# xxxxxxyp/Light-3D-Unet-Front

Measured on AMD Instinct MI355X. Metric: train patches/sec (48³, bs=4/GPU) at 1/2/4/8 MI355X + fwd ms/patch, higher is better.
Workload: dtype fp32; 1 GPU; Lightweight3DUNet 16->32->64->128 train step (fwd+FocalTversky+bwd+AdamW), 48^3 patches; batch_per_gpu=4, global_batch=4, ftl_mode=exact, parallelism=single, graph=True

## Files before the change

### include/l3u.h

```cpp
#ifndef L3U_H
#define L3U_H

#include <hip/hip_runtime.h>

#ifdef __cplusplus
extern "C" {
#endif

typedef unsigned short l3u_bf16;

#define L3U_ABI_VERSION 5
int l3u_abi_version(void);

typedef struct l3u_norm_src {
  const float* stat_part;
  int nsb;
  int layer;
  const float* gamma;
  const float* beta;
  float drop_p;
  unsigned long long seed;
  const int* step;
  float* rec_out;
  const float* rank1;
// ... 76 lines not shown
                    float drop_p, unsigned long long seed, const int* step, int layer, float* rec,
                    int N, int C, hipStream_t stream);
int l3u_norm_act_nblocks(int S);
int l3u_norm_act_fwd(const float* y2, long long y2_nstride, const float* rec2,
                     const l3u_norm_src* src2, const float* r, long long r_nstride,
                     const float* rec_r, const l3u_norm_src* src_r, int shortcut, float* out,
                     long long out_nstride, int N, int C, int S, hipStream_t stream);
int l3u_norm_act_pool_fwd(const float* y2, long long y2_nstride, const float* rec2,
                          const l3u_norm_src* src2, const float* r, long long r_nstride,
                          const float* rec_r, const l3u_norm_src* src_r, int shortcut, float* out,
                          long long out_nstride, float* pooled, long long pooled_nstride,
                          unsigned char* idx, int N, int C, int D, int H, int W,
                          hipStream_t stream);
int l3u_norm_act_bwd_reduce(const float* dout, long long dout_nstride, const float* out,
                            long long out_nstride, const float* y2, long long y2_nstride,
                            const float* rec2, const float* r, long long r_nstride,
                            const float* rec_r, double* part, int N, int C, int S,
                            hipStream_t stream);
int l3u_norm_act_bwd_reduce_r1(const float* dz, long long dz_nstride, const float* dscale,
                               const float* out, long long out_nstride, const float* y2,
                               long long y2_nstride, const float* rec2, const float* r,
                               long long r_nstride, const float* rec_r, double* part, int N, int C,
                               int S, hipStream_t stream);
int l3u_norm_act_bwd_reduce_up(const float* dskip, long long dskip_nstride, const float* dpool,
                               long long dpool_nstride, const unsigned char* idx, const float* out,
                               long long out_nstride, const float* y2, long long y2_nstride,
                               const float* rec2, const float* r, long long r_nstride,
                               const float* rec_r, double* part, int N, int C, int D, int H, int W,
                               hipStream_t stream);
int l3u_norm_act_bwd_apply(const float* dout, long long dout_nstride, const float* out,
                           long long out_nstride, const float* y2, long long y2_nstride,
                           const float* rec2, const float* r, long long r_nstride,
                           const float* rec_r, const double* part, float* dy2,
                           long long dy2_nstride, float* dr, long long dr_nstride, int N, int C,
                           int S, hipStream_t stream);
int l3u_norm_act_bwd(const float* dout, long long dout_nstride, const float* out,
                     long long out_nstride, const float* y2, long long y2_nstride,
                     const float* rec2, const float* r, long long r_nstride, const float* rec_r,
                     double* part, float* dy2, long long dy2_nstride, float* dr,
                     long long dr_nstride, int N, int C, int S, hipStream_t stream);
int l3u_norm_act_bwd_up(const float* dskip, long long dskip_nstride, const float* dpool,
                        long long dpool_nstride, const unsigned char* idx, const float* out,
                        long long out_nstride, const float* y2, long long y2_nstride,
                        const float* rec2, const float* r, long long r_nstride,
                        const float* rec_r, double* part, float* dy2, long long dy2_nstride,
                        float* dr, long long dr_nstride, int N, int C, int D, int H, int W,
// ... 439 lines not shown
```

### light-3d-unet-front_amd/csrc/misc.hip

```cpp
#include "common.h"
#ifdef L3U_STAMP
#include <vector>
#endif
using namespace l3u;

typedef float f4 __attribute__((ext_vector_type(4)));

namespace {

template <typename T>
__global__ __launch_bounds__(256) void maxpool2_fwd_kernel(
    const T* __restrict__ x, long long xns, T* __restrict__ y, long long yns,
    unsigned char* __restrict__ idx, int C, int D, int H, int W) {
  L3U_STAMP_SCOPE(401);
  const int Do = D / 2, Ho = H / 2, Wo = W / 2;
  const long long So = (long long)Do * Ho * Wo, Si = (long long)D * H * W;
  const int nc = blockIdx.y, c = nc % C, n = nc / C;
  const T* xp = x + (long long)n * xns + (long long)c * Si;
  T* yp = y + (long long)n * yns + (long long)c * So;
  unsigned char* ip = idx + (long long)nc * So;
  for (long long o = blockIdx.x * 256ll + threadIdx.x; o < So; o += (long long)gridDim.x * 256) {
    const int ox = (int)(o % Wo), t = (int)(o / Wo), oy = t % Ho, oz = t / Ho;
    const T* b = xp + ((long long)(2 * oz) * H + 2 * oy) * W + 2 * ox;
    float best = ld1(b);
// ... 85 lines not shown
#pragma unroll
  for (int q = 0; q < 4; ++q) {
    if (i0 + q < S) {
      const float tv = VEC ? tv4[q] : t[(long long)n * S + i0 + q];
      spt = fmaf(pv[q], tv, spt);
      sp += pv[q];
      st += tv;
      if (L4) se += bce_term(pv[q], tv);
    }
  }
  spt = block_sum256(spt, red);
  sp = block_sum256(sp, red);
  st = block_sum256(st, red);
  if (L4) se = block_sum256(se, red);
  if (threadIdx.x == 0) {
    float* o = ftl_part + ((long long)n * gridDim.x + blockIdx.x) * (L4 ? 4 : 3);
    o[0] = spt;
    o[1] = sp;
    o[2] = st;
    if (L4) o[3] = se;
  }
}

struct FtlCoef { double loss, A, B; };

L3U_DEV FtlCoef ftl_coef(const double* sums, double alpha, double beta, double gamma, double smooth) {
  const double tp = sums[0], fp = sums[1] - sums[0], fn = sums[2] - sums[0];
  const double dn = tp + alpha * fn + beta * fp + smooth;
  const double ti = (tp + smooth) / dn;
  const double one_m = 1.0 - ti;
  FtlCoef r;
  r.loss = pow(one_m, gamma);
  const double pre = -gamma * pow(one_m, gamma - 1.0) / (dn * dn);
  r.A = pre * (dn - (tp + smooth) * (1.0 - alpha));
  r.B = pre * (-(tp + smooth) * beta);
  return r;
}

L3U_DEV void ftl_lane_sums(const float* __restrict__ part, int nb, double& a, double& b, double& c) {
  const int l = threadIdx.x & 63;
  a = b = c = 0.0;
  constexpr int B = 8;
  for (int i = l; i < nb; i += B * 64) {
    float va[B], vb[B], vc[B];
#pragma unroll
    for (int u = 0; u < B; ++u) {
      const int j = min(i + u * 64, nb - 1);
      va[u] = part[j * 3];
      vb[u] = part[j * 3 + 1];
      vc[u] = part[j * 3 + 2];
    }
#pragma unroll
    for (int u = 0; u < B; ++u) {
      const bool ok = i + u * 64 < nb;
      a += ok ? va[u] : 0.f;
      b += ok ? vb[u] : 0.f;
      c += ok ? vc[u] : 0.f;
    }
  }
  a = wave_sum_d(a);
  b = wave_sum_d(b);
  c = wave_sum_d(c);
}

L3U_DEV void loss4_lane_sums(const float* __restrict__ part, int nb, double* sm) {
  const int l = threadIdx.x & 63;
  double a = 0.0, b = 0.0, c = 0.0, d = 0.0;
  constexpr int B = 8;
  for (int i = l; i < nb; i += B * 64) {
    float va[B], vb[B], vc[B], vd[B];
#pragma unroll
    for (int u = 0; u < B; ++u) {
      const int j = min(i + u * 64, nb - 1);
      va[u] = part[j * 4];
      vb[u] = part[j * 4 + 1];
      vc[u] = part[j * 4 + 2];
      vd[u] = part[j * 4 + 3];
    }
#pragma unroll
    for (int u = 0; u < B; ++u) {
      const bool ok = i + u * 64 < nb;
      a += ok ? va[u] : 0.f;
      b += ok ? vb[u] : 0.f;
      c += ok ? vc[u] : 0.f;
      d += ok ? vd[u] : 0.f;
    }
// ... 59 lines not shown
    }
#pragma unroll
    for (int c = 0; c < 32; ++c) {
      hv[c] = f4{0.f, 0.f, 0.f, 0.f};
      if (c < C && i0 < S) hv[c] = ldv4(hp + (long long)c * S + i0);
    }
  }
  float cA = 0.f, cB = 0.f, cE = 0.f;
  if (L4 && dp == nullptr) {
    double sm[4];
    if (fpart != nullptr) {
      loss4_lane_sums(fpart, fnp, sm);
    } else {
      sm[0] = sums[0]; sm[1] = sums[1]; sm[2] = sums[2]; sm[3] = sums[3];
    }
    const Loss4Coef r = loss4_coef(sm, fam);
    const double s = gscale ? (double)gscale[0] : 1.0;
    cA = (float)(r.A * s);
    cB = (float)(r.B * s);
    cE = (float)(r.E * s);
    if (loss && blockIdx.x == 0 && blockIdx.y == 0 && threadIdx.x == 0) loss[0] = (float)r.loss;
  }
  if (!L4 && dp == nullptr) {
    double sm[3];
    if (fpart != nullptr) {
      ftl_lane_sums(fpart, fnp, sm[0], sm[1], sm[2]);
    } else {
      sm[0] = sums[0]; sm[1] = sums[1]; sm[2] = sums[2];
    }
    const FtlCoef r = ftl_coef(sm, alpha, beta, gamma, smooth);
    const double s = gscale ? (double)gscale[0] : 1.0;
    cA = (float)(r.A * s);
    cB = (float)(r.B * s);
    if (loss && blockIdx.x == 0 && blockIdx.y == 0 && threadIdx.x == 0) loss[0] = (float)r.loss;
  }
  f4 dz = {0.f, 0.f, 0.f, 0.f};
#pragma unroll
  for (int q = 0; q < 4; ++q) {
    if (i0 + q < S) {
      const float pv = VEC ? pv4[q] : p[o + i0 + q];
      const float gs = VEC ? gv4[q] : (dp ? dp[o + i0 + q] : t[o + i0 + q]);
      const float g = dp ? gs : (L4 ? loss4_grad(cA - cB, cB, cE, pv, gs) : fmaf(cA - cB, gs, cB));
      dz[q] = g * pv * (1.f - pv);
    }
  }
  float acc[33];
#pragma unroll
  for (int c = 0; c < 33; ++c) acc[c] = 0.f;
  acc[32] = (dz[0] + dz[1]) + (dz[2] + dz[3]);
  if (dz_only) {
    if (VEC) {
      if (i0 < S) stv4(dhp + i0, dz);
    } else {
#pragma unroll
      for (int q = 0; q < 4; ++q)
        if (i0 + q < S) st1(dhp + i0 + q, dz[q]);
    }
  }
#pragma unroll
  for (int c = 0; c < 32; ++c) {
    if (c < C) {
      if (VEC) {
        if (i0 < S) {
          const f4 hc = hv[VEC ? c : 0];
          acc[c] = fmaf(dz[0], hc[0], fmaf(dz[1], hc[1], fmaf(dz[2], hc[2], dz[3] * hc[3])));
          if (!dz_only) stv4(dhp + (long long)c * S + i0, w[c] * dz);
        }
      } else {
#pragma unroll
        for (int q = 0; q < 4; ++q)
          if (i0 + q < S) {
            acc[c] = fmaf(dz[q], ld1(hp + (long long)c * S + i0 + q), acc[c]);
            if (!dz_only) st1(dhp + (long long)c * S + i0 + q, w[c] * dz[q]);
          }
      }
    }
  }
  const int wv = threadIdx.x >> 6, l = threadIdx.x & 63;
#pragma unroll
  for (int c = 0; c < 33; ++c) {
    if (c < C || c == 32) {
      const double r = wave_sum_d((double)acc[c]);
      if (l == 0) redd[wv * (C + 1) + (c == 32 ? C : c)] = r;
    }
  }
  __syncthreads();
  if (threadIdx.x <= C) {
    const int tt = threadIdx.x;
// ... 856 lines not shown
```

### light-3d-unet-front_amd/csrc/norm.hip

```cpp
#include "common.h"
using namespace l3u;

typedef float f4 __attribute__((ext_vector_type(4)));

namespace {

__global__ __launch_bounds__(256) void in_finalize_kernel(l3u_norm_src src, int NC, int C) {
  L3U_STAMP_SCOPE(301);
  const int wid = blockIdx.x * 4 + (threadIdx.x >> 6), l = threadIdx.x & 63;
  if (wid >= NC) return;
  float r[kRec];
  finalize_record(src, wid / C, wid % C, C, r);
  if (l == 0) {
    float* o = src.rec_out + (long long)wid * kRec;
#pragma unroll
    for (int i = 0; i < kRec; ++i) o[i] = r[i];
  }
}

template <typename T, bool VEC, bool HAS_SRC, bool RK = false>
__global__ __launch_bounds__(256) void norm_act_fwd_kernel(
    const T* __restrict__ y2, long long y2ns, const float* __restrict__ rec2, l3u_norm_src src2,
    const T* __restrict__ r, long long rns, const float* __restrict__ recr, l3u_norm_src srcr,
    int shortcut, T* __restrict__ out, long long ons, int C, int S) {
// ... 116 lines not shown
      stv4(op + off, v[j]);
      v[j] = round_to(v[j], (const T*)nullptr);
    }
    float b0 = v[0][0], b1 = v[0][2];
    int i0 = 0, i1 = 0;
#pragma unroll
    for (int j = 0; j < 4; ++j)
#pragma unroll
      for (int dx = 0; dx < 2; ++dx) {
        if (j == 0 && dx == 0) continue;
        const float u0 = v[j][dx], u1 = v[j][2 + dx];
        if (u0 > b0 || u0 != u0) { b0 = u0; i0 = 2 * j + dx; }
        if (u1 > b1 || u1 != u1) { b1 = u1; i1 = 2 * j + dx; }
      }
    stv2(pp + 2 * o, f2_t{b0, b1});
    ip[o] = (unsigned short)(i0 | (i1 << 8));
  }
}

#ifndef L3U_NABR_U
#define L3U_NABR_U 2
#endif
constexpr int kNabrU = L3U_NABR_U;
template <typename T, bool VEC, bool RK = false, bool PL = false>
__global__ __launch_bounds__(256) void norm_act_bwd_reduce_kernel(
    const float* __restrict__ dout, long long dns, const T* __restrict__ out, long long ons,
    const T* __restrict__ y2, long long y2ns, const float* __restrict__ rec2,
    const T* __restrict__ r, long long rns, const float* __restrict__ recr,
    double* __restrict__ part, int N, int C, int S, const float* __restrict__ dscale = nullptr,
    const float* __restrict__ dpool = nullptr, long long dpns = 0,
    const unsigned char* __restrict__ pidx = nullptr, int H = 0, int W = 0) {
  L3U_STAMP_SCOPE(304);
  kargs_now(dout, dns, out, ons, y2, y2ns, rec2, r, rns, recr, part, N, C, S, dscale, dpool, dpns,
            pidx, H, W);
  __shared__ double red[4];
  const int nc = blockIdx.y, c = nc % C, n = nc / C, nb = gridDim.x;
  const float m2 = rec2[(long long)nc * kRec + 0], rs2 = rec2[(long long)nc * kRec + 1];
  float mr = 0.f, rsr = 1.f, rks = 1.f;
  if (recr) {
    mr = recr[(long long)nc * kRec + 0]; rsr = recr[(long long)nc * kRec + 1];
    rks = recr[(long long)nc * kRec + 7];
  }
  constexpr bool rk = RK;
  const long long co = (long long)c * S;
  const float* dp = dout + (long long)n * dns + (dscale ? 0 : co);
  const float dsc = dscale ? dscale[c] : 1.f;
  const T* op = out + (long long)n * ons + co;
  const T* yp = y2 + (long long)n * y2ns + co;
  const T* rp = r + (long long)n * (rk ? -rns : rns) + (rk ? 0ll : co);
  double s0 = 0.0, s1 = 0.0, s2 = 0.0;
  if (VEC) {
    constexpr int U = kNabrU;
    const int step = nb * 1024;
    const T* rq = recr ? rp : op;
    for (int i0 = (blockIdx.x * 256 + threadIdx.x) * 4; i0 < S; i0 += U * step) {
      f4 ov[U], dv[U], yv[U], rv[U];
      UnpoolTap pt[U];
      int zz[U], yy[U];
#pragma unroll
      for (int u = 0; u < U; ++u) {
        const int i = min(i0 + u * step, S - 4);
        ov[u] = ldv4(op + i);
        dv[u] = ldv4(dp + i);
        yv[u] = ldv4(yp + i);
        rv[u] = ldv4(rq + i);
      }
      if constexpr (PL) {
#pragma unroll
        for (int u = 0; u < U; ++u) {
          const int i = min(i0 + u * step, S - 4);
          const int HW = H * W, z = fdiv(i, HW, 1.f / HW), rm = i - z * HW, y = fdiv(rm, W, 1.f / W);
          zz[u] = z; yy[u] = y;
          pt[u] = unpool_tap(dpool + (long long)n * dpns + (long long)c * (S / 8),
                             pidx + (long long)nc * (S / 8), z, y, rm - y * W, H, W);
        }
      }
      __builtin_amdgcn_sched_barrier(0);
#pragma unroll
      for (int u = 0; u < U; ++u) {
        dv[u] = dsc * dv[u];
        if constexpr (PL) dv[u] = unpool_apply(dv[u], pt[u], zz[u], yy[u]);
        if (rk) rv[u] = mul_rn(rv[u], rks);
      }
#pragma unroll
      for (int u = 0; u < U; ++u) {
        const bool in = u == 0 || i0 + u * step < S;
#pragma unroll
        for (int q = 0; q < 4; ++q) {
          const float g = dv[u][q] * lrelu_d(ov[u][q]);
          const double t1 = (double)g * ((yv[u][q] - m2) * rs2);
          const double t2 = (double)g * ((rv[u][q] - mr) * rsr);
          s0 = in ? s0 + g : s0;
          s1 = in ? s1 + t1 : s1;
          if (recr) s2 = in ? s2 + t2 : s2;
        }
      }
    }
  } else {
    for (int i = blockIdx.x * 256 + threadIdx.x; i < S; i += nb * 256) {
      const float g = (dscale ? dsc * ld1(dp + i) : ld1(dp + i)) * lrelu_d(ld1(op + i));
      s0 += g;
      s1 += (double)g * ((ld1(yp + i) - m2) * rs2);
      if (recr) s2 += (double)g * (((rk ? mul_rn(rks, ld1(rp + i)) : ld1(rp + i)) - mr) * rsr);
    }
  }
  s0 = block_sum256d(s0, red);
  s1 = block_sum256d(s1, red);
  s2 = block_sum256d(s2, red);
  if (threadIdx.x == 0) {
// ... 331 lines not shown
                             const float* rec_r, double* part, int N, int C, int S,
                             hipStream_t stream, const float* dscale = nullptr,
                             const float* dpool = nullptr, long long dpns = 0,
                             const unsigned char* pidx = nullptr, int H = 0, int W = 0) {
  L3U_REQUIRE(N > 0 && C > 0 && S > 0);
  L3U_REQUIRE(r_nstride >= 0 || (sizeof(T) == 4 && rec_r != nullptr));
  const bool vec = S % 4 == 0 && dout_nstride % 4 == 0 && out_nstride % 4 == 0 &&
                   y2_nstride % 4 == 0 && r_nstride % 4 == 0;
  L3U_REQUIRE(dpool == nullptr || (vec && pidx && H % 2 == 0 && W % 4 == 0 && (S / (H * W)) % 2 == 0 &&
                                   dpns % 2 == 0 && ((uintptr_t)dpool & 7) == 0));
  dim3 grid(elem_blocks(S), N * C);
  L3U_REQUIRE(r_nstride >= 0 || vec);
#define NABR(RK_, PL_) hipLaunchKernelGGL((norm_act_bwd_reduce_kernel<T, true, RK_, PL_>), grid, dim3(256), 0, \
      stream, dout, dout_nstride, out, out_nstride, y2, y2_nstride, rec2, r, r_nstride, rec_r, part, N, C, S, \
      dscale, dpool, dpns, pidx, H, W)
  if (r_nstride < 0) {
    if constexpr (sizeof(T) == 4) { if (dpool) NABR(true, true); else NABR(true, false); }
  } else if (vec) { if (dpool) NABR(false, true); else NABR(false, false); }
#undef NABR
  else hipLaunchKernelGGL((norm_act_bwd_reduce_kernel<T, false>), grid, dim3(256), 0, stream, dout, dout_nstride, out, out_nstride, y2, y2_nstride, rec2, r, r_nstride, rec_r, part, N, C, S, dscale);
  L3U_CHECK_LAUNCH();
}

template <typename T>
int norm_act_bwd_apply_impl(const float* dout, long long dout_nstride, const T* out,
                            long long out_nstride, const T* y2, long long y2_nstride,
                            const float* rec2, const T* r, long long r_nstride,
                            const float* rec_r, const double* part, float* dy2,
                            long long dy2_nstride, float* dr, long long dr_nstride, int N, int C,
                            int S, hipStream_t stream) {
  L3U_REQUIRE(N > 0 && C > 0 && S > 0);
  L3U_REQUIRE(r_nstride >= 0);
  const bool vec = S % 4 == 0 && dout_nstride % 4 == 0 && out_nstride % 4 == 0 &&
                   y2_nstride % 4 == 0 && r_nstride % 4 == 0 && dy2_nstride % 4 == 0 &&
                   dr_nstride % 4 == 0;
  const int npart = elem_blocks(S);
  dim3 grid(npart, N * C);
  if (vec) hipLaunchKernelGGL((norm_act_bwd_apply_kernel<T, true>), grid, dim3(256), 0, stream, dout, dout_nstride, out, out_nstride, y2, y2_nstride, rec2, r, r_nstride, rec_r, part, npart, dy2, dy2_nstride, dr, dr_nstride, N, C, S);
  else hipLaunchKernelGGL((norm_act_bwd_apply_kernel<T, false>), grid, dim3(256), 0, stream, dout, dout_nstride, out, out_nstride, y2, y2_nstride, rec2, r, r_nstride, rec_r, part, npart, dy2, dy2_nstride, dr, dr_nstride, N, C, S);
  L3U_CHECK_LAUNCH();
}

template <typename T>
int norm_act_bwd_impl(const float* dout, long long dout_nstride, const T* out,
                      long long out_nstride, const T* y2, long long y2_nstride,
                      const float* rec2, const T* r, long long r_nstride, const float* rec_r,
// ... 41 lines not shown
    int C, int D, int H, int W, hipStream_t stream)
L3U_TWIN(l3u_norm_act_pool_fwd, P_NAP, norm_act_pool_fwd_impl(bp(y2), y2_nstride, rec2, src2, bp(r),
         r_nstride, rec_r, src_r, shortcut, bp(out), out_nstride, bp(pooled), pooled_nstride, idx, N,
         C, D, H, W, stream))
#define P_NBR(TT) (const float* dout, long long dout_nstride, const TT* out, long long out_nstride,   \
    const TT* y2, long long y2_nstride, const float* rec2, const TT* r, long long r_nstride,        \
    const float* rec_r, double* part, int N, int C, int S, hipStream_t stream)
L3U_TWIN(l3u_norm_act_bwd_reduce, P_NBR, norm_act_bwd_reduce_impl(dout, dout_nstride, bp(out),
         out_nstride, bp(y2), y2_nstride, rec2, bp(r), r_nstride, rec_r, part, N, C, S, stream))
#define P_NBR1(TT) (const float* dz, long long dz_nstride, const float* dscale, const TT* out,        \
    long long out_nstride, const TT* y2, long long y2_nstride, const float* rec2, const TT* r,       \
    long long r_nstride, const float* rec_r, double* part, int N, int C, int S, hipStream_t stream)
#define P_NBRU(TT) (const float* dskip, long long dskip_nstride, const float* dpool,                  \
    long long dpool_nstride, const unsigned char* idx, const TT* out, long long out_nstride,         \
    const TT* y2, long long y2_nstride, const float* rec2, const TT* r, long long r_nstride,        \
    const float* rec_r, double* part, int N, int C, int D, int H, int W, hipStream_t stream)
L3U_TWIN(l3u_norm_act_bwd_reduce_up, P_NBRU, dpool == nullptr ? (int)hipErrorInvalidValue :
         norm_act_bwd_reduce_impl(dskip, dskip_nstride, bp(out), out_nstride, bp(y2), y2_nstride, rec2,
         bp(r), r_nstride, rec_r, part, N, C, D * H * W, stream, nullptr, dpool, dpool_nstride, idx, H,
         W))
L3U_TWIN(l3u_norm_act_bwd_reduce_r1, P_NBR1, dscale == nullptr ? (int)hipErrorInvalidValue :
         norm_act_bwd_reduce_impl(dz, dz_nstride, bp(out), out_nstride, bp(y2), y2_nstride, rec2, bp(r),
         r_nstride, rec_r, part, N, C, S, stream, dscale))
#define P_NBA(TT) (const float* dout, long long dout_nstride, const TT* out, long long out_nstride,   \
    const TT* y2, long long y2_nstride, const float* rec2, const TT* r, long long r_nstride,        \
    const float* rec_r, const double* part, float* dy2, long long dy2_nstride, float* dr,          \
    long long dr_nstride, int N, int C, int S, hipStream_t stream)
L3U_TWIN(l3u_norm_act_bwd_apply, P_NBA, norm_act_bwd_apply_impl(dout, dout_nstride, bp(out),
         out_nstride, bp(y2), y2_nstride, rec2, bp(r), r_nstride, rec_r, part, dy2, dy2_nstride,
         dr, dr_nstride, N, C, S, stream))
#define P_NB1(TT) (const float* dout, long long dout_nstride, const TT* out, long long out_nstride,   \
    const TT* y2, long long y2_nstride, const float* rec2, const TT* r, long long r_nstride,        \
    const float* rec_r, double* part, float* dy2, long long dy2_nstride, float* dr,                 \
    long long dr_nstride,                                                                            \
    int N, int C, int S, hipStream_t stream)
L3U_TWIN(l3u_norm_act_bwd, P_NB1, norm_act_bwd_impl(dout, dout_nstride, bp(out), out_nstride,
         bp(y2), y2_nstride, rec2, bp(r), r_nstride, rec_r, part, dy2, dy2_nstride, dr,
         dr_nstride, N, C, S, stream))
#define P_NB1U(TT) (const float* dskip, long long dskip_nstride, const float* dpool,                 \
    long long dpool_nstride, const unsigned char* idx, const TT* out, long long out_nstride,         \
    const TT* y2, long long y2_nstride, const float* rec2, const TT* r, long long r_nstride,        \
    const float* rec_r, double* part, float* dy2, long long dy2_nstride, float* dr,                 \
    long long dr_nstride, int N, int C, int D, int H, int W, hipStream_t stream)
L3U_TWIN(l3u_norm_act_bwd_up, P_NB1U, dpool == nullptr ? (int)hipErrorInvalidValue :
         norm_act_bwd_impl(dskip, dskip_nstride, bp(out), out_nstride, bp(y2), y2_nstride, rec2,
         bp(r), r_nstride, rec_r, part, dy2, dy2_nstride, dr, dr_nstride, N, C, D * H * W, stream,
// ... 8 lines not shown
```

### light-3d-unet-front_amd/light_unet/_native.py

```python
import ctypes
import os
import warnings

import torch

_HERE = os.path.dirname(os.path.abspath(__file__))
LIB_PATH = os.environ.get(
    "L3U_LIB", os.path.join(os.path.dirname(_HERE), "lib", "libl3u_hip.so"))

ABI_VERSION = 5

P = ctypes.c_void_p
I = ctypes.c_int
L = ctypes.c_longlong
F = ctypes.c_float
D = ctypes.c_double
U64 = ctypes.c_ulonglong

_FAM = [D] * 9

_SIGS = {
    "l3u_abi_version": [],
    "l3u_dw3_nchunk": [I, I, I, I, I],
    "l3u_dw3_fwd": [P, L, P, P, P, P, L, I, I, I, I, I, P],
# ... 48 lines not shown
    "l3u_gconv3_fwd": [P, L, P, P, P, L, P, I, I, I, I, I, I, I, P],
    "l3u_gconv3_bwd_data": [P, L, P, P, P, L, P, L, I, P, I, I, I, I, I, I, I, P],
    "l3u_gconv3_bwd_weight": [P, L, P, L, P, P, I, I, I, I, I, I, I, P],
    "l3u_counter_add": [P, I, P],
    "l3u_cast_f32_bf16": [P, P, L, P],
    "l3u_box_copy": [P, L, I, I, I, P, L, I, I, I, I, I, I, I, I, P],
    "l3u_ccl_nchunks": [L],
    "l3u_aug_patches": [P, I, I, I, I, P, P, P, P, P, P],
    "l3u_aug_draw": [P, P, I, D, U64, P, I, I, I, I, P, P, P, P, P],
    "l3u_ccl_label": [P, F, P, P, P, I, I, I, P],
    "l3u_ccl_stats": [P, P, P, P, I, I, I, I, P],
    "l3u_ccl_pairs": [P, P, I, P, L, P],
    "l3u_ccl_label_b": [P, F, P, P, P, I, I, I, I, P],
    "l3u_ccl_stats_b": [P, P, P, P, I, I, I, I, I, I, P],
    "l3u_ccl_lv_max_levels": [L, L],
    "l3u_thr_levels": [P, P, P, P, I, P, P, P, L, P],
    "l3u_ccl_label_lv": [P, I, I, P, P, P, P, I, I, I, P],
    "l3u_ccl_stats_lv": [P, P, P, P, I, I, I, I, I, P],
    "l3u_ccl_pairs_lv": [P, P, I, P, P, I, L, P],
    "l3u_cast_bf16_f32": [P, P, L, P],
    "l3u_outconv_bwd_dz": [P, P, P, P, D, D, D, D, P, P, L, P, P, L, P, P, I, I, I, P],
    "l3u_outconv_bwd_ftl_dz": [P, P, P, I, D, D, D, D, P, P, L, P, P, L, P, P, I, I, I, P],
    "l3u_norm_act_bwd_reduce_r1": [P, L, P, P, L, P, L, P, P, L, P, P, I, I, I, P],
    "l3u_pw_bwd_tail_r1": [P, L, P, P, L, P, L, P, P, I, I, P, L, P, P, L, I, P, I, I, I, I, P],
    "l3u_norm_act_bwd_reduce_up": [P, L, P, L, P, P, L, P, L, P, P, L, P, P, I, I, I, I, I, P],
    "l3u_pw_bwd_tail_up": [P, L, P, L, P, P, L, P, L, P, P, I, I, P, L, P, P, L, I, P, I, I, I, I, I, I,
                           P],
    "l3u_dwpw_supported": [I, I, I, I, I, I],
    "l3u_dw3_bwd_rank1": [I, I, I, I, I],
    "l3u_dwpw_stat_nsb": [I, I, I, I, I],
    "l3u_dwpw_fwd": [P, L, P, P, P, P, P, L, P, P, P, L, P, P, L, I, I, I, I, I, I, P],
    "l3u_loss4_sums": [P, P, L, P, P, P],
    "l3u_loss4_reduce": [P, I, P, P],
    "l3u_loss4_value": [P] + _FAM + [P, P],
    "l3u_loss4_bwd": [P, P, L, P] + _FAM + [P, I, P, P],
    "l3u_outconv_fwd_loss4": [P, L, P, P, P, P, P, I, I, I, P],
    "l3u_outconv_bwd_loss4": [P, P, P] + _FAM + [P, P, L, P, P, L, P, P, I, I, I, P],
    "l3u_outconv_bwd_loss4_dz": [P, P, P] + _FAM + [P, P, L, P, P, L, P, P, I, I, I, P],
    "l3u_outconv_bwd_loss4p": [P, P, P, I] + _FAM + [P, P, L, P, P, L, P, P, I, I, I, P],
    "l3u_outconv_bwd_loss4p_dz": [P, P, P, I] + _FAM + [P, P, L, P, P, L, P, P, I, I, I, P],
    "l3u_pp_select_ws_bytes": [],
    "l3u_pp_select": [P, I, L, I, L, L, L, L, P, P, P],
    "l3u_pp_normalize": [P, I, P, D, D, D, P, P, P, I, I, I, P],
    "l3u_pp_pack": [P, I, I, D, P, I, I, I, P],
    "l3u_pp_unpack": [P, P, I, I, I, I, P],
    "l3u_pp_morph_max_iters": [I],
# ... 139 lines not shown
```

### light-3d-unet-front_amd/light_unet/engine.py

```python
import math
import os

import torch

from . import _native as nat

F32 = 4
_FRONT = os.environ.get("L3U_FRONT", "1") != "0"
_PAIR_PW = os.environ.get("L3U_PAIR_PW", "1") != "0"
_TAIL_FUSE = os.environ.get("L3U_TAIL_FUSE", "1") != "0"
_SEG_CAPS = tuple(int(v) for v in os.environ.get("L3U_SEG_CAPS", "128,64,32").split(","))
_SEG_SHORT = tuple(int(v) for v in os.environ.get("L3U_SEG_SHORT", "32:256").split(":"))
_DWPW = os.environ.get("L3U_DWPW", "1") != "0"
_PAIR_BWD = os.environ.get("L3U_PAIR_BWD", "1") != "0"
_PAIR_TAIL_MAX_S = int(os.environ.get("L3U_PAIR_TAIL_MAX_S", str(48 ** 3)))
_PAIR_TAIL_NARROW = os.environ.get("L3U_PAIR_TAIL_NARROW", "1") != "0"
_DWPW_MIN_S = int(os.environ.get("L3U_DWPW_MIN_S", "65536"))
_RANK1 = os.environ.get("L3U_RANK1", "1") != "0"
_POOLFOLD = os.environ.get("L3U_POOLFOLD", "1") != "0"
_FRONT_R1 = os.environ.get("L3U_FRONT_R1", "1") != "0"
_FUSE_ADAMW = os.environ.get("L3U_FUSE_ADAMW", "1") != "0"


_SEG_SORT = os.environ.get("L3U_SEG_SORT", "1") != "0"


def _seg_rounds(it):
    src, cnt, ist, tst, ln, _, _, f64 = it
    vec = not f64 and tst == 1 and ln % 4 == 0 and ist % 4 == 0 and src % 4 == 0
    tp = 256 // (ln // 4) if vec else 256 // ln
    return -(-(-(-cnt // tp)) // 8)


def _items_cover_once(items, numel):
    cnt = torch.zeros(numel, dtype=torch.int32)
    for it in items:
        if it[6]:
            return False
        cnt[it[5]:it[5] + it[4]] += 1
    return bool((cnt == 1).all())


class V:
    __slots__ = ("t", "off", "ns", "C", "scale", "pool")

    def __init__(self, t, off, ns, C, scale=None, pool=None):
        self.t, self.off, self.ns, self.C, self.scale = t, off, ns, C, scale
        self.pool = pool

    @property
    def p(self):
        return self.t.data_ptr() + self.t.element_size() * self.off

    @property
    def sns(self):
        return -self.ns if self.scale is not None else self.ns


def conv_kinds(cin, cout, use_depthwise_separable=True, use_grouped=True, groups=8):
    if use_depthwise_separable:
        return ("ds", 0), ("ds", 0)
    k1 = ("grouped", groups) if (use_grouped and groups > 1 and cin >= groups and cout >= groups) \
        else ("dense", 1)
    k2 = ("grouped", groups) if (use_grouped and groups > 1 and cout >= groups) else ("dense", 1)
    return k1, k2


def _conv_params(pre, kind, cin, cout):
    if kind[0] == "ds":
        return [(pre + "depthwise.weight", (cin, 1, 3, 3, 3)),
# ... 537 lines not shown
        else:
            nat.call("l3u_reduce_segments", self.bwd_arena.ptr(0), items.data_ptr(),
                     items.shape[0], gflat.data_ptr(), nat.stream())
        return dx

    def _backward_impl(self, flat, gflat, sv, dp, need_dx, ftl=None, family=None):
        N = sv["N"]
        dims, S = sv["dims"], sv["S"]
        c0, c1, c2, c3 = self.enc
        dev = sv["p"].device
        e = lambda *s: self._empty(*s, device=dev)
        st = nat.stream()
        A = self.bwd_arena
        h = sv["h"]
        up3 = sv["blk"]["up3.res_block."]
        r1 = _RANK1 and self.kinds["up3.res_block."][0][0] == "ds" and \
            self._tail_fusable(up3, up3["x"].C, c0, S[0])
        sfx = "_dz" if r1 else ""
        dh = e(N, 1, S[0]) if r1 else e(N, c0, S[0])
        dhns = S[0] if r1 else c0 * S[0]
        nb = nat.query("l3u_outconv_nblocks", S[0])
        po = A.alloc(2 * N * nb * (c0 + 1))
        loss_ptr = None
        if dp is not None:
            g = (dp.data_ptr(), None, None, 0.0, 0.0, 0.0, 0.0, None)
            self._call("l3u_outconv_bwd" + sfx, g[0], sv["p"].data_ptr(), *g[1:], h.p, h.ns,
                       self._w(flat, "out_conv.weight"), dh.data_ptr(), dhns, A.ptr(po),
                       loss_ptr, N, c0, S[0], st)
        elif family is not None:
            t, sums = ftl[:2]
            if len(ftl) > 3 and ftl[3] is not None:
                loss_ptr = ftl[3].data_ptr()
            tail = (None, h.p, h.ns, self._w(flat, "out_conv.weight"), dh.data_ptr(), dhns,
                    A.ptr(po), loss_ptr, N, c0, S[0], st)
            if sums is None:
                self._call("l3u_outconv_bwd_loss4p" + sfx, sv["p"].data_ptr(), t.data_ptr(),
                           ftl[4].data_ptr(), ftl[5], *family, *tail)
            else:
                self._call("l3u_outconv_bwd_loss4" + sfx, sv["p"].data_ptr(), t.data_ptr(),
                           sums.data_ptr(), *family, *tail)
        else:
            t, sums, (alpha, beta, gamma, smooth) = ftl[:3]
            if len(ftl) > 3 and ftl[3] is not None:
                loss_ptr = ftl[3].data_ptr()
            if sums is None:
                fpart, fnp = ftl[4], ftl[5]
                self._call("l3u_outconv_bwd_ftl" + sfx, sv["p"].data_ptr(), t.data_ptr(),
                           fpart.data_ptr(), fnp, alpha, beta, gamma, smooth, None, h.p, h.ns,
                           self._w(flat, "out_conv.weight"), dh.data_ptr(), dhns, A.ptr(po),
                           loss_ptr, N, c0, S[0], st)
            else:
                self._call("l3u_outconv_bwd" + sfx, None, sv["p"].data_ptr(), t.data_ptr(),
                           sums.data_ptr(), alpha, beta, gamma, smooth, None, h.p, h.ns,
                           self._w(flat, "out_conv.weight"), dh.data_ptr(), dhns, A.ptr(po),
                           loss_ptr, N, c0, S[0], st)
        self._seg(po // 2, N * nb, c0 + 1, 1, c0, "out_conv.weight", f64=1)
        self._seg(po // 2 + c0, N * nb, c0 + 1, 1, 1, "out_conv.bias", f64=1)
        dcat3, dcat2, dcat1 = e(N, 2 * c0, S[0]), e(N, 2 * c1, S[1]), e(N, 2 * c2, S[2])
        dcats = {0: dcat3, 1: dcat2, 2: dcat1}
        dout = V(dh, 0, dhns, c0, self._w(flat, "out_conv.weight") if r1 else None)
        up_specs = [("up3.", c0, 0, 2), ("up2.", c1, 1, 1), ("up1.", c2, 2, 0)]
        for up, co, lvl, uidx in up_specs:
            dcat = dcats[lvl]
            self._block_bwd(flat, up + "res_block.", sv["blk"][up + "res_block."], dout,
                            V(dcat, 0, 2 * co * S[lvl], 2 * co), st, dev)
            prev, _ = sv["ups"][uidx]
            ci = prev.C
            d, hh, w = dims[lvl + 1]
            dprev = e(N, ci, S[lvl + 1])
            dY, dYns = dcat.data_ptr(), 2 * co * S[lvl]
            pad = self.up_pad(dims[lvl + 1], dims[lvl])
            if pad is not None:
                dup = self._f32(N, co, 8 * S[lvl + 1], device=dev)
                self._call32("l3u_box_copy", dY, dYns, *dims[lvl], dup.data_ptr(), co * 8 * S[lvl + 1],
                             2 * d, 2 * hh, 2 * w, *[-o for o in pad], N, co, st)
                dY, dYns = dup.data_ptr(), co * 8 * S[lvl + 1]
            npf = nat.query("l3u_convt_bwd_fused_nparts", N, ci, co, d, hh, w)
            if npf > 0:
                pw, pb = A.alloc(npf * ci * co * 8), A.alloc(npf * co)
                self._call("l3u_convt_bwd_fused", dY, dYns, prev.p, prev.ns,
                           self._w(flat, up + "up.weight"), dprev.data_ptr(), ci * S[lvl + 1],
                           A.ptr(pw), A.ptr(pb), N, ci, co, d, hh, w, st)
                self._seg(pw, npf, ci * co * 8, 1, ci * co * 8, up + "up.weight")
# ... 43 lines not shown
                and cout <= 32 and nat.query("l3u_pw_bwd_supported", cout, cout, S)
                and nat.query("l3u_pw_bwd_supported", cout, cin, S))

    @staticmethod
    def _tail_one_up(sv, S):
        return (nat.query("l3u_norm_act_nblocks", S) == 1 and S <= 2048
                and (sv["r"] if sv["shortcut"] else sv["x"]).scale is None)

    def _tail_bwd(self, pre, sv, dout, dxv, N, cout, S, st, dev, fused=False):
        A = self.bwd_arena
        out, recs = sv["out"], sv["recs"]
        rec_r, rec2 = recs[0].data_ptr(), recs[2].data_ptr()
        shortcut = sv["shortcut"]
        rv = sv["r"] if shortcut else sv["x"]
        y2 = sv["y2"]
        nb = nat.query("l3u_norm_act_nblocks", S)
        pn = A.alloc(2 * cout * N * nb * 3)
        pnd = pn // 2
        self._seg(pnd + 1, N * nb, 3, N * nb * 3, cout, pre + "norm2.weight", f64=1)
        self._seg(pnd + 0, N * nb, 3, N * nb * 3, cout, pre + "norm2.bias", f64=1)
        if fused:
            self._seg(pnd + 2, N * nb, 3, N * nb * 3, cout, pre + "shortcut.1.weight", f64=1)
            self._seg(pnd + 0, N * nb, 3, N * nb * 3, cout, pre + "shortcut.1.bias", f64=1)
            if dout.scale is not None:
                self._call("l3u_norm_act_bwd_reduce_r1", dout.p, dout.ns, dout.scale, out.p, out.ns,
                           y2.data_ptr(), cout * S, rec2, rv.p, rv.sns, rec_r, A.ptr(pn), N, cout, S,
                           st)
            elif dout.pool is not None:
                dpool, idx, (d, h, w) = dout.pool
                self._call("l3u_norm_act_bwd_reduce_up", dout.p, dout.ns, dpool.data_ptr(),
                           cout * (S // 8), idx.data_ptr(), out.p, out.ns, y2.data_ptr(), cout * S,
                           rec2, rv.p, rv.sns, rec_r, A.ptr(pn), N, cout, d, h, w, st)
            else:
                self._call("l3u_norm_act_bwd_reduce", dout.p, dout.ns, out.p, out.ns, y2.data_ptr(),
                           cout * S, rec2, rv.p, rv.sns, rec_r, A.ptr(pn), N, cout, S, st)
            return pn, nb
        assert dout.scale is None and (dout.pool is None or nb == 1), "a formed-on-load output " \
            "gradient needs the fused block tail or a one-launch plane"
        assert rv.scale is None, "a rank-1 residual needs the fused block tail"
        dy2 = self._empty(N, cout, S, device=dev)
        if shortcut:
            dr = self._empty(N, cout, S, device=dev)
            drv = V(dr, 0, cout * S, cout)
            self._seg(pnd + 2, N * nb, 3, N * nb * 3, cout, pre + "shortcut.1.weight", f64=1)
            self._seg(pnd + 0, N * nb, 3, N * nb * 3, cout, pre + "shortcut.1.bias", f64=1)
        else:
            drv = dxv
# ... 231 lines not shown
```

Before: 3782 patches/s.

## Fold focal-Tversky output-conv backward into the up3 norm-act backward reduce

Adds a fused kernel variant that computes the FTL loss coefficients, the sigmoid/out-conv dz, and the out-conv weight/bias partial sums inside the up3 block's norm-act backward reduce pass. It reads p and t directly instead of a materialized dz, so the separate out-conv backward launch and its extra full-resolution read/write pass are meant to go away. It also adds per-tile wave reductions, shared memory and a block barrier per loop iteration, and FTL helpers move into a shared header. It is gated by an env flag, fp32 only, and requires S >= 32768.

```diff
diff --git a/include/l3u.h b/include/l3u.h
--- a/include/l3u.h
+++ b/include/l3u.h
@@ -122,6 +122,15 @@
                                long long y2_nstride, const float* rec2, const float* r,
                                long long r_nstride, const float* rec_r, double* part, int N, int C,
                                int S, hipStream_t stream);
+int l3u_norm_act_bwd_reduce_r1_ftl(const float* p, const float* t, const float* ftl_part,
+                                   int ftl_nparts, const double* sums, double alpha, double beta,
+                                   double gamma, double smooth, const float* gscale,
+                                   const float* w_out, float* dz, long long dz_nstride,
+                                   double* oc_part, float* loss, const float* out,
+                                   long long out_nstride, const float* y2, long long y2_nstride,
+                                   const float* rec2, const float* r, long long r_nstride,
+                                   const float* rec_r, double* part, int N, int C, int S,
+                                   hipStream_t stream);
 int l3u_norm_act_bwd_reduce_up(const float* dskip, long long dskip_nstride, const float* dpool,
                                long long dpool_nstride, const unsigned char* idx, const float* out,
                                long long out_nstride, const float* y2, long long y2_nstride,
diff --git a/light-3d-unet-front_amd/csrc/ftl.h b/light-3d-unet-front_amd/csrc/ftl.h
--- /dev/null
+++ b/light-3d-unet-front_amd/csrc/ftl.h
@@ -0,0 +1,71 @@
+#pragma once
+#include "common.h"
+
+namespace l3u {
+
+struct FtlCoef { double loss, A, B; };
+
+L3U_DEV FtlCoef ftl_coef(const double* sums, double alpha, double beta, double gamma, double smooth) {
+  const double tp = sums[0], fp = sums[1] - sums[0], fn = sums[2] - sums[0];
+  const double dn = tp + alpha * fn + beta * fp + smooth;
+  const double ti = (tp + smooth) / dn;
+  const double one_m = 1.0 - ti;
+  FtlCoef r;
+  r.loss = pow(one_m, gamma);
+  const double pre = -gamma * pow(one_m, gamma - 1.0) / (dn * dn);
+  r.A = pre * (dn - (tp + smooth) * (1.0 - alpha));
+  r.B = pre * (-(tp + smooth) * beta);
+  return r;
+}
+
+L3U_DEV void ftl_lane_sums(const float* __restrict__ part, int nb, double& a, double& b, double& c) {
+  const int l = threadIdx.x & 63;
+  a = b = c = 0.0;
+  constexpr int B = 8;
+  for (int i = l; i < nb; i += B * 64) {
+    float va[B], vb[B], vc[B];
+#pragma unroll
+    for (int u = 0; u < B; ++u) {
+      const int j = min(i + u * 64, nb - 1);
+      va[u] = part[j * 3];
+      vb[u] = part[j * 3 + 1];
+      vc[u] = part[j * 3 + 2];
+    }
+#pragma unroll
+    for (int u = 0; u < B; ++u) {
+      const bool ok = i + u * 64 < nb;
+      a += ok ? va[u] : 0.f;
+      b += ok ? vb[u] : 0.f;
+      c += ok ? vc[u] : 0.f;
+    }
+  }
+  a = wave_sum_d(a);
+  b = wave_sum_d(b);
+  c = wave_sum_d(c);
+}
+
+L3U_DEV double ftl_scaled_coef(const float* __restrict__ fpart, int fnp, const double* __restrict__ sums,
+                               double alpha, double beta, double gamma, double smooth,
+                               const float* __restrict__ gscale, float& cA, float& cB) {
+  double sm[3];
+  if (fpart != nullptr) {
+    ftl_lane_sums(fpart, fnp, sm[0], sm[1], sm[2]);
+  } else {
+    sm[0] = sums[0]; sm[1] = sums[1]; sm[2] = sums[2];
+  }
+  const FtlCoef r = ftl_coef(sm, alpha, beta, gamma, smooth);
+  const double s = gscale ? (double)gscale[0] : 1.0;
+  cA = (float)(r.A * s);
+  cB = (float)(r.B * s);
+  return r.loss;
+}
+
+L3U_DEV float sigmoid_bwd(float g, float pv) { return g * pv * (1.f - pv); }
+L3U_DEV float ftl_dz(float cAB, float cB, float pv, float tv) { return sigmoid_bwd(fmaf(cAB, tv, cB), pv); }
+
+L3U_DEV float outconv_wgrad4(f4_t dz, f4_t hc) {
+  return fmaf(dz[0], hc[0], fmaf(dz[1], hc[1], fmaf(dz[2], hc[2], dz[3] * hc[3])));
+}
+L3U_DEV float outconv_bgrad4(f4_t dz) { return (dz[0] + dz[1]) + (dz[2] + dz[3]); }
+
+}
diff --git a/light-3d-unet-front_amd/csrc/misc.hip b/light-3d-unet-front_amd/csrc/misc.hip
--- a/light-3d-unet-front_amd/csrc/misc.hip
+++ b/light-3d-unet-front_amd/csrc/misc.hip
@@ -1,4 +1,5 @@
 #include "common.h"
+#include "ftl.h"
 #ifdef L3U_STAMP
 #include <vector>
 #endif
@@ -131,46 +132,6 @@
   }
 }
 
-struct FtlCoef { double loss, A, B; };
-
-L3U_DEV FtlCoef ftl_coef(const double* sums, double alpha, double beta, double gamma, double smooth) {
-  const double tp = sums[0], fp = sums[1] - sums[0], fn = sums[2] - sums[0];
-  const double dn = tp + alpha * fn + beta * fp + smooth;
-  const double ti = (tp + smooth) / dn;
-  const double one_m = 1.0 - ti;
-  FtlCoef r;
-  r.loss = pow(one_m, gamma);
-  const double pre = -gamma * pow(one_m, gamma - 1.0) / (dn * dn);
-  r.A = pre * (dn - (tp + smooth) * (1.0 - alpha));
-  r.B = pre * (-(tp + smooth) * beta);
-  return r;
-}
-
-L3U_DEV void ftl_lane_sums(const float* __restrict__ part, int nb, double& a, double& b, double& c) {
-  const int l = threadIdx.x & 63;
-  a = b = c = 0.0;
-  constexpr int B = 8;
-  for (int i = l; i < nb; i += B * 64) {
-    float va[B], vb[B], vc[B];
-#pragma unroll
-    for (int u = 0; u < B; ++u) {
-      const int j = min(i + u * 64, nb - 1);
-      va[u] = part[j * 3];
-      vb[u] = part[j * 3 + 1];
-      vc[u] = part[j * 3 + 2];
-    }
-#pragma unroll
-    for (int u = 0; u < B; ++u) {
-      const bool ok = i + u * 64 < nb;
-      a += ok ? va[u] : 0.f;
-      b += ok ? vb[u] : 0.f;
-      c += ok ? vc[u] : 0.f;
-    }
-  }
-  a = wave_sum_d(a);
-  b = wave_sum_d(b);
-  c = wave_sum_d(c);
-}
 
 L3U_DEV void loss4_lane_sums(const float* __restrict__ part, int nb, double* sm) {
   const int l = threadIdx.x & 63;
@@ -276,17 +237,8 @@
     if (loss && blockIdx.x == 0 && blockIdx.y == 0 && threadIdx.x == 0) loss[0] = (float)r.loss;
   }
   if (!L4 && dp == nullptr) {
-    double sm[3];
-    if (fpart != nullptr) {
-      ftl_lane_sums(fpart, fnp, sm[0], sm[1], sm[2]);
-    } else {
-      sm[0] = sums[0]; sm[1] = sums[1]; sm[2] = sums[2];
-    }
-    const FtlCoef r = ftl_coef(sm, alpha, beta, gamma, smooth);
-    const double s = gscale ? (double)gscale[0] : 1.0;
-    cA = (float)(r.A * s);
-    cB = (float)(r.B * s);
-    if (loss && blockIdx.x == 0 && blockIdx.y == 0 && threadIdx.x == 0) loss[0] = (float)r.loss;
+    const double lv = ftl_scaled_coef(fpart, fnp, sums, alpha, beta, gamma, smooth, gscale, cA, cB);
+    if (loss && blockIdx.x == 0 && blockIdx.y == 0 && threadIdx.x == 0) loss[0] = (float)lv;
   }
   f4 dz = {0.f, 0.f, 0.f, 0.f};
 #pragma unroll
@@ -294,14 +246,14 @@
     if (i0 + q < S) {
       const float pv = VEC ? pv4[q] : p[o + i0 + q];
       const float gs = VEC ? gv4[q] : (dp ? dp[o + i0 + q] : t[o + i0 + q]);
-      const float g = dp ? gs : (L4 ? loss4_grad(cA - cB, cB, cE, pv, gs) : fmaf(cA - cB, gs, cB));
-      dz[q] = g * pv * (1.f - pv);
+      dz[q] = dp ? sigmoid_bwd(gs, pv)
+                 : (L4 ? sigmoid_bwd(loss4_grad(cA - cB, cB, cE, pv, gs), pv) : ftl_dz(cA - cB, cB, pv, gs));
     }
   }
   float acc[33];
 #pragma unroll
   for (int c = 0; c < 33; ++c) acc[c] = 0.f;
-  acc[32] = (dz[0] + dz[1]) + (dz[2] + dz[3]);
+  acc[32] = outconv_bgrad4(dz);
   if (dz_only) {
     if (VEC) {
       if (i0 < S) stv4(dhp + i0, dz);
@@ -316,8 +268,7 @@
     if (c < C) {
       if (VEC) {
         if (i0 < S) {
-          const f4 hc = hv[VEC ? c : 0];
-          acc[c] = fmaf(dz[0], hc[0], fmaf(dz[1], hc[1], fmaf(dz[2], hc[2], dz[3] * hc[3])));
+          acc[c] = outconv_wgrad4(dz, hv[VEC ? c : 0]);
           if (!dz_only) stv4(dhp + (long long)c * S + i0, w[c] * dz);
         }
       } else {
diff --git a/light-3d-unet-front_amd/csrc/norm.hip b/light-3d-unet-front_amd/csrc/norm.hip
--- a/light-3d-unet-front_amd/csrc/norm.hip
+++ b/light-3d-unet-front_amd/csrc/norm.hip
@@ -1,4 +1,5 @@
 #include "common.h"
+#include "ftl.h"
 using namespace l3u;
 
 typedef float f4 __attribute__((ext_vector_type(4)));
@@ -162,18 +163,31 @@
 #define L3U_NABR_U 2
 #endif
 constexpr int kNabrU = L3U_NABR_U;
-template <typename T, bool VEC, bool RK = false, bool PL = false>
+struct FtlFold {
+  const float *p, *t, *fpart;
+  int fnp;
+  const double* sums;
+  double alpha, beta, gamma, smooth;
+  const float* gscale;
+  float* dz;
+  long long dzns;
+  double* ocpart;
+  float* loss;
+};
+template <typename T, bool VEC, bool RK = false, bool PL = false, bool FT = false>
 __global__ __launch_bounds__(256) void norm_act_bwd_reduce_kernel(
     const float* __restrict__ dout, long long dns, const T* __restrict__ out, long long ons,
     const T* __restrict__ y2, long long y2ns, const float* __restrict__ rec2,
     const T* __restrict__ r, long long rns, const float* __restrict__ recr,
     double* __restrict__ part, int N, int C, int S, const float* __restrict__ dscale = nullptr,
     const float* __restrict__ dpool = nullptr, long long dpns = 0,
-    const unsigned char* __restrict__ pidx = nullptr, int H = 0, int W = 0) {
+    const unsigned char* __restrict__ pidx = nullptr, int H = 0, int W = 0,
+    FtlFold ft = FtlFold()) {
   L3U_STAMP_SCOPE(304);
   kargs_now(dout, dns, out, ons, y2, y2ns, rec2, r, rns, recr, part, N, C, S, dscale, dpool, dpns,
             pidx, H, W);
   __shared__ double red[4];
+  __shared__ double redo[FT ? 2 * kNabrU * 2 * 4 : 1];
   const int nc = blockIdx.y, c = nc % C, n = nc / C, nb = gridDim.x;
   const float m2 = rec2[(long long)nc * kRec + 0], rs2 = rec2[(long long)nc * kRec + 1];
   float mr = 0.f, rsr = 1.f, rks = 1.f;
@@ -189,19 +203,34 @@
   const T* yp = y2 + (long long)n * y2ns + co;
   const T* rp = r + (long long)n * (rk ? -rns : rns) + (rk ? 0ll : co);
   double s0 = 0.0, s1 = 0.0, s2 = 0.0;
+  float cAB = 0.f, cB = 0.f;
+  if constexpr (FT) {
+    float cA;
+    const double lv = ftl_scaled_coef(ft.fpart, ft.fnp, ft.sums, ft.alpha, ft.beta, ft.gamma,
+                                      ft.smooth, ft.gscale, cA, cB);
+    cAB = cA - cB;
+    if (ft.loss && blockIdx.x == 0 && blockIdx.y == 0 && threadIdx.x == 0) ft.loss[0] = (float)lv;
+  }
   if (VEC) {
     constexpr int U = kNabrU;
     const int step = nb * 1024;
     const T* rq = recr ? rp : op;
-    for (int i0 = (blockIdx.x * 256 + threadIdx.x) * 4; i0 < S; i0 += U * step) {
-      f4 ov[U], dv[U], yv[U], rv[U];
+    int tile = blockIdx.x, par = 0;
+    for (int i0 = (blockIdx.x * 256 + threadIdx.x) * 4; (FT ? i0 - (int)threadIdx.x * 4 : i0) < S;
+         i0 += U * step) {
+      f4 ov[U], dv[U], yv[U], rv[U], tv[U];
       UnpoolTap pt[U];
       int zz[U], yy[U];
 #pragma unroll
       for (int u = 0; u < U; ++u) {
         const int i = min(i0 + u * step, S - 4);
         ov[u] = ldv4(op + i);
-        dv[u] = ldv4(dp + i);
+        if constexpr (FT) {
+          dv[u] = ldv4(ft.p + (long long)n * S + i);
+          tv[u] = ldv4(ft.t + (long long)n * S + i);
+        } else {
+          dv[u] = ldv4(dp + i);
+        }
         yv[u] = ldv4(yp + i);
         rv[u] = ldv4(rq + i);
       }
@@ -216,6 +245,33 @@
         }
       }
       __builtin_amdgcn_sched_barrier(0);
+      if constexpr (FT) {
+        const int nbo = (S + 1023) / 1024, wv = threadIdx.x >> 6;
+#pragma unroll
+        for (int u = 0; u < U; ++u) {
+          const bool in = i0 + u * step < S;
+          f4 dz;
+#pragma unroll
+          for (int q = 0; q < 4; ++q) dz[q] = ftl_dz(cAB, cB, dv[u][q], tv[u][q]);
+          if (c == 0 && in) stv4(ft.dz + (long long)n * ft.dzns + i0 + u * step, dz);
+          const double wa = wave_sum_d((double)(in ? outconv_wgrad4(dz, ov[u]) : 0.f));
+          const double wb = c == 0 ? wave_sum_d((double)(in ? outconv_bgrad4(dz) : 0.f)) : 0.0;
+          if ((threadIdx.x & 63) == 0) {
+            redo[((par * U + u) * 2 + 0) * 4 + wv] = wa;
+            redo[((par * U + u) * 2 + 1) * 4 + wv] = wb;
+          }
+          dv[u] = dz;
+        }
+        __syncthreads();
+        if (threadIdx.x < U && tile + (int)threadIdx.x * nb < nbo) {
+          const double* q = redo + (par * U + threadIdx.x) * 2 * 4;
+          double* o = ft.ocpart + ((long long)n * nbo + tile + (int)threadIdx.x * nb) * (C + 1);
+          o[c] = (q[0] + q[1]) + (q[2] + q[3]);
+          if (c == 0) o[C] = (q[4] + q[5]) + (q[6] + q[7]);
+        }
+        tile += U * nb;
+        par ^= 1;
+      }
 #pragma unroll
       for (int u = 0; u < U; ++u) {
         dv[u] = dsc * dv[u];
@@ -224,7 +280,7 @@
       }
 #pragma unroll
       for (int u = 0; u < U; ++u) {
-        const bool in = u == 0 || i0 + u * step < S;
+        const bool in = (!FT && u == 0) || i0 + u * step < S;
 #pragma unroll
         for (int q = 0; q < 4; ++q) {
           const float g = dv[u][q] * lrelu_d(ov[u][q]);
@@ -602,6 +658,27 @@
   L3U_CHECK_LAUNCH();
 }
 
+int norm_act_bwd_reduce_ftl_impl(const FtlFold& ft, const float* dscale, const float* out,
+                                 long long out_nstride, const float* y2, long long y2_nstride,
+                                 const float* rec2, const float* r, long long r_nstride,
+                                 const float* rec_r, double* part, int N, int C, int S,
+                                 hipStream_t stream) {
+  L3U_REQUIRE(N > 0 && C > 0 && S > 0 && ft.p && ft.t && ft.dz && ft.ocpart && dscale && out && y2 &&
+              rec2 && r && rec_r && part);
+  L3U_REQUIRE((ft.sums != nullptr) != (ft.fpart != nullptr) && (ft.fpart == nullptr || ft.fnp > 0));
+  L3U_REQUIRE(S % 4 == 0 && ft.dzns % 4 == 0 && out_nstride % 4 == 0 && y2_nstride % 4 == 0 &&
+              r_nstride % 4 == 0 &&
+              (((uintptr_t)ft.p | (uintptr_t)ft.t | (uintptr_t)ft.dz | (uintptr_t)out | (uintptr_t)y2 |
+                (uintptr_t)r) & 15) == 0);
+  dim3 grid(elem_blocks(S), N * C);
+#define NABF(RK_) hipLaunchKernelGGL((norm_act_bwd_reduce_kernel<float, true, RK_, false, true>), grid, \
+      dim3(256), 0, stream, ft.dz, ft.dzns, out, out_nstride, y2, y2_nstride, rec2, r, r_nstride, rec_r, part, \
+      N, C, S, dscale, (const float*)nullptr, 0ll, (const unsigned char*)nullptr, 0, 0, ft)
+  if (r_nstride < 0) NABF(true); else NABF(false);
+#undef NABF
+  L3U_CHECK_LAUNCH();
+}
+
 template <typename T>
 int norm_act_bwd_apply_impl(const float* dout, long long dout_nstride, const T* out,
                             long long out_nstride, const T* y2, long long y2_nstride,
@@ -689,6 +766,17 @@
 L3U_TWIN(l3u_norm_act_bwd_reduce_r1, P_NBR1, dscale == nullptr ? (int)hipErrorInvalidValue :
          norm_act_bwd_reduce_impl(dz, dz_nstride, bp(out), out_nstride, bp(y2), y2_nstride, rec2, bp(r),
          r_nstride, rec_r, part, N, C, S, stream, dscale))
+extern "C" int l3u_norm_act_bwd_reduce_r1_ftl(
+    const float* p, const float* t, const float* ftl_part, int ftl_nparts, const double* sums,
+    double alpha, double beta, double gamma, double smooth, const float* gscale, const float* w_out,
+    float* dz, long long dz_nstride, double* oc_part, float* loss, const float* out,
+    long long out_nstride, const float* y2, long long y2_nstride, const float* rec2, const float* r,
+    long long r_nstride, const float* rec_r, double* part, int N, int C, int S, hipStream_t stream) {
+  const FtlFold ft{p, t, ftl_part, ftl_nparts, sums, alpha, beta, gamma, smooth, gscale, dz, dz_nstride,
+                   oc_part, loss};
+  return norm_act_bwd_reduce_ftl_impl(ft, w_out, out, out_nstride, y2, y2_nstride, rec2, r, r_nstride,
+                                      rec_r, part, N, C, S, stream);
+}
 #define P_NBA(TT) (const float* dout, long long dout_nstride, const TT* out, long long out_nstride,   \
     const TT* y2, long long y2_nstride, const float* rec2, const TT* r, long long r_nstride,        \
     const float* rec_r, const double* part, float* dy2, long long dy2_nstride, float* dr,          \
diff --git a/light-3d-unet-front_amd/light_unet/_native.py b/light-3d-unet-front_amd/light_unet/_native.py
--- a/light-3d-unet-front_amd/light_unet/_native.py
+++ b/light-3d-unet-front_amd/light_unet/_native.py
@@ -94,6 +94,8 @@
     "l3u_outconv_bwd_dz": [P, P, P, P, D, D, D, D, P, P, L, P, P, L, P, P, I, I, I, P],
     "l3u_outconv_bwd_ftl_dz": [P, P, P, I, D, D, D, D, P, P, L, P, P, L, P, P, I, I, I, P],
     "l3u_norm_act_bwd_reduce_r1": [P, L, P, P, L, P, L, P, P, L, P, P, I, I, I, P],
+    "l3u_norm_act_bwd_reduce_r1_ftl": [P, P, P, I, P, D, D, D, D, P, P, P, L, P, P, P, L, P, L, P, P, L,
+                                       P, P, I, I, I, P],
     "l3u_pw_bwd_tail_r1": [P, L, P, P, L, P, L, P, P, I, I, P, L, P, P, L, I, P, I, I, I, I, P],
     "l3u_norm_act_bwd_reduce_up": [P, L, P, L, P, P, L, P, L, P, P, L, P, P, I, I, I, I, I, P],
     "l3u_pw_bwd_tail_up": [P, L, P, L, P, P, L, P, L, P, P, I, I, P, L, P, P, L, I, P, I, I, I, I, I, I,
diff --git a/light-3d-unet-front_amd/light_unet/engine.py b/light-3d-unet-front_amd/light_unet/engine.py
--- a/light-3d-unet-front_amd/light_unet/engine.py
+++ b/light-3d-unet-front_amd/light_unet/engine.py
@@ -17,6 +17,8 @@
 _PAIR_TAIL_NARROW = os.environ.get("L3U_PAIR_TAIL_NARROW", "1") != "0"
 _DWPW_MIN_S = int(os.environ.get("L3U_DWPW_MIN_S", "65536"))
 _RANK1 = os.environ.get("L3U_RANK1", "1") != "0"
+_OUTFOLD = os.environ.get("L3U_OUTFOLD", "1") != "0"
+_OUTFOLD_MIN_S = max(32768, int(os.environ.get("L3U_OUTFOLD_MIN_S", "32768")))
 _POOLFOLD = os.environ.get("L3U_POOLFOLD", "1") != "0"
 _FRONT_R1 = os.environ.get("L3U_FRONT_R1", "1") != "0"
 _FUSE_ADAMW = os.environ.get("L3U_FUSE_ADAMW", "1") != "0"
@@ -42,10 +44,11 @@
 
 
 class V:
-    __slots__ = ("t", "off", "ns", "C", "scale", "pool")
+    __slots__ = ("t", "off", "ns", "C", "scale", "pool", "fold")
 
     def __init__(self, t, off, ns, C, scale=None, pool=None):
         self.t, self.off, self.ns, self.C, self.scale = t, off, ns, C, scale
+        self.fold = None
         self.pool = pool
 
     @property
@@ -629,7 +632,17 @@
         nb = nat.query("l3u_outconv_nblocks", S[0])
         po = A.alloc(2 * N * nb * (c0 + 1))
         loss_ptr = None
-        if dp is not None:
+        fold = None
+        if (_OUTFOLD and r1 and dp is None and family is None and not self.bf16
+                and S[0] >= _OUTFOLD_MIN_S and S[0] % 4 == 0 and h.p == up3["out"].p):
+            t, sums, (alpha, beta, gamma, smooth) = ftl[:3]
+            if len(ftl) > 3 and ftl[3] is not None:
+                loss_ptr = ftl[3].data_ptr()
+            fold = (sv["p"].data_ptr(), t.data_ptr(), ftl[4].data_ptr() if sums is None else None,
+                    ftl[5] if sums is None else 0, None if sums is None else sums.data_ptr(), alpha,
+                    beta, gamma, smooth, None, self._w(flat, "out_conv.weight"), dh.data_ptr(), dhns,
+                    A.ptr(po), loss_ptr)
+        elif dp is not None:
             g = (dp.data_ptr(), None, None, 0.0, 0.0, 0.0, 0.0, None)
             self._call("l3u_outconv_bwd" + sfx, g[0], sv["p"].data_ptr(), *g[1:], h.p, h.ns,
                        self._w(flat, "out_conv.weight"), dh.data_ptr(), dhns, A.ptr(po),
@@ -666,6 +679,7 @@
         dcat3, dcat2, dcat1 = e(N, 2 * c0, S[0]), e(N, 2 * c1, S[1]), e(N, 2 * c2, S[2])
         dcats = {0: dcat3, 1: dcat2, 2: dcat1}
         dout = V(dh, 0, dhns, c0, self._w(flat, "out_conv.weight") if r1 else None)
+        dout.fold = fold
         up_specs = [("up3.", c0, 0, 2), ("up2.", c1, 1, 1), ("up1.", c2, 2, 0)]
         for up, co, lvl, uidx in up_specs:
             dcat = dcats[lvl]
@@ -755,7 +769,10 @@
         if fused:
             self._seg(pnd + 2, N * nb, 3, N * nb * 3, cout, pre + "shortcut.1.weight", f64=1)
             self._seg(pnd + 0, N * nb, 3, N * nb * 3, cout, pre + "shortcut.1.bias", f64=1)
-            if dout.scale is not None:
+            if dout.fold is not None:
+                self._call("l3u_norm_act_bwd_reduce_r1_ftl", *dout.fold, out.p, out.ns, y2.data_ptr(),
+                           cout * S, rec2, rv.p, rv.sns, rec_r, A.ptr(pn), N, cout, S, st)
+            elif dout.scale is not None:
                 self._call("l3u_norm_act_bwd_reduce_r1", dout.p, dout.ns, dout.scale, out.p, out.ns,
                            y2.data_ptr(), cout * S, rec2, rv.p, rv.sns, rec_r, A.ptr(pn), N, cout, S,
                            st)
```

Result: no change. 3797 patches/s (median of 6 runs) (+0.4%).
